# chanzuckerberg/saber

Measured on AMD Instinct MI355X. Metric: EM slices/sec (1024^2, Hiera-L), higher is better.
Workload: dtype bf16; 1 GPU; 1024x1024 uint16 EM slice -> prep.prepare -> SAM2 AMG (Hiera-L, cfgAMG defaults: npoints=32, crop_n_layers=2 -> 21 crops, 3072 grid prompts + 9216 m2m refinements, multimask) -> dedup/sort -> uint16 label plane; BASELINE configs[1]; weights=seeded synthetic Hiera-L (no checkpoint offline), slices_per_rank=22, engine_handles_per_gpu=2, parallelism=single GPU

## Files before the change

### include/saber_amd_kernels.h

```cpp
#ifndef SABER_AMD_KERNELS_H
#define SABER_AMD_KERNELS_H
#include <stdint.h>
#ifdef __cplusplus
extern "C" {
#endif

const char* saber_k_last_error(void);
int saber_k_init(int device_id);

int saber_k_gemm(const uint16_t* A, const uint16_t* W, const float* bias, const float* res, float* out_f32, uint16_t* out_bf16,
                 int M, int N, int K, int act, int act_last, int pool4, int res_shift, int res_mod, void* stream);

int saber_k_gemm_ld(const uint16_t* A, int lda, const uint16_t* W, int ldw, int w_kpad, const float* bias, const float* res, float* out_f32,
                    uint16_t* out_bf16, int M, int N, int K, int act, void* stream);

int saber_k_gemm_rowln(const uint16_t* A, int lda, const uint16_t* W, int ldw, const float* bias, const float* res, float* out_f32,
                       uint16_t* out_bf16, const float* ln_gamma, const float* ln_beta, float ln_eps, uint16_t* ln_out, int M, int N, int K,
                       void* stream);

int saber_k_mlp_rowln(const uint16_t* A, int lda, const uint16_t* W1, int ldw1, const float* b1, const uint16_t* W2, int ldw2, const float* b2,
                      const float* res, float* out_f32, uint16_t* out_bf16, const float* ln_gamma, const float* ln_beta, float ln_eps,
                      uint16_t* ln_out, int M, int C, void* stream);

int saber_k_layernorm(const float* x, const float* gamma, const float* beta, float eps, float* out_f32, uint16_t* out_bf16,
                      int rows, int C, int act, void* stream);

int saber_k_hiera_attention(const uint16_t* qkv, uint16_t* out, int n_windows, int nk, int heads, int q_pool, void* stream);
int saber_k_hiera_attention_ex(const uint16_t* qkv, uint16_t* out, int n_windows, int nk, int heads, int head_dim, int q_pool,
                               const uint8_t* key_mask, void* stream);

int saber_k_dec_attention(const float* q, const float* k, const float* v, uint16_t* out, int B, int nq, int nk, int heads, int hd,
                          int k_shared, void* stream);

int saber_k_prepare(const void* img, int dtype, int H, int W, float* out, float* ws_dev, uint32_t* minmax_dev, void* stream);

int saber_k_mask_post(const float* lowres, int n, int crop_x0, int crop_y0, int crop_w, int crop_h, int H, int W, float thr,
                      float offset, uint32_t* bits, int32_t* stats, void* stream);
// ... 92 lines not shown
```

### saber_amd/_lib.py

```python
import ctypes as C
import os
import subprocess

_HERE = os.path.dirname(os.path.abspath(__file__))
LIB_PATH = os.path.join(_HERE, "libsaber_amd.so")
CSRC = os.path.join(_HERE, "csrc")


class SaberAmdError(RuntimeError):
    pass


class SaberRangeError(SaberAmdError):
    """SABER_ERR_RANGE: the engine's overflow sentinel found NaN / inf in the 16-bit arithmetic (include/saber_amd.h:
    saber_engine_check_finite) - with fp16 operands, an activation beyond 65 504.  The call's results are invalid."""


SABER_OK, SABER_ERR_INVALID, SABER_ERR_STATE, SABER_ERR_HIP, SABER_ERR_CAPACITY, SABER_ERR_RANGE = 0, -1, -2, -3, -4, -5


def build(verbose: bool = False) -> str:
    r = subprocess.run(["make", "-C", CSRC, "-j8"], capture_output=True, text=True)
    if r.returncode != 0:
        raise SaberAmdError("building libsaber_amd.so failed:\n" + r.stdout[-4000:] + r.stderr[-4000:])
# ... 76 lines not shown
    "saber_classifier_predict": (_i, [_vp, _vp, _i, _i, _vp, _i, _i, _vp, _vp]),
    "saber_classifier_predict_bits": (_i, [_vp, _vp, _i, _i, _vp, _i, C.POINTER(_i), _i, _i, _vp, _vp]),
    "saber_classifier_head": (_i, [_vp, _vp, _i, _vp, _vp]),
    "saber_classifier_get_crops": (_i, [_vp, _i, _vp, _vp, _vp]),
    "saber_profile_begin": (_i, [_vp]),
    "saber_profile_end": (_i, [_vp, C.POINTER(ProfileClass), _i]),
    "saber_encoder_flops": (C.c_double, [_vp]),
    "saber_decoder_flops_per_prompt": (C.c_double, []),
    "saber_k_last_error": (C.c_char_p, []),
    "saber_k_init": (_i, [_i]),
    "saber_k_gemm": (_i, [_vp, _vp, _vp, _vp, _vp, _vp, _i, _i, _i, _i, _i, _i, _i, _i, _vp]),
    "saber_k_gemm_ld": (_i, [_vp, _i, _vp, _i, _i, _vp, _vp, _vp, _vp, _i, _i, _i, _i, _vp]),
    "saber_k_gemm_rowln": (_i, [_vp, _i, _vp, _i, _vp, _vp, _vp, _vp, _vp, _vp, _f, _vp, _i, _i, _i, _vp]),
    "saber_k_mlp_rowln": (_i, [_vp, _i, _vp, _i, _vp, _vp, _i, _vp, _vp, _vp, _vp, _vp, _vp, _f, _vp, _i, _i, _vp]),
    "saber_k_layernorm": (_i, [_vp, _vp, _vp, _f, _vp, _vp, _i, _i, _i, _vp]),
    "saber_k_hiera_attention": (_i, [_vp, _vp, _i, _i, _i, _i, _vp]),
    "saber_k_hiera_attention_ex": (_i, [_vp, _vp, _i, _i, _i, _i, _i, _vp, _vp]),
    "saber_k_dec_attention": (_i, [_vp, _vp, _vp, _vp, _i, _i, _i, _i, _i, _i, _vp]),
    "saber_k_prepare": (_i, [_vp, _i, _i, _i, _vp, _vp, _vp, _vp]),
    "saber_k_mask_post": (_i, [_vp, _i, _i, _i, _i, _i, _i, _i, _f, _f, _vp, _vp, _vp]),
    "saber_k_perm_index": (_i, [_i, _i, _i]),
    "saber_k_set_operand_type": (_i, [_i]),
    "saber_k_stream_create_cu_range": (_i, [_i, _i, C.POINTER(_vp)]),
    "saber_k_stream_destroy": (_i, [_vp]),
    "saber_k_host_f32_to_f16": (None, [_vp, _vp, C.c_int64]),
    "saber_k_dec_i2t": (_i, [_vp, C.c_int64, _vp, _vp, _vp, _f, _vp, _vp, _vp, _vp, _vp, _f, _vp, _i, _vp]),
    "saber_k_dec_i2t16": (_i, [_vp, C.c_int64, _vp, _vp, _vp, _f, _vp, _vp, _vp, _vp, _vp, _f, _vp, _i, _i, _vp]),
    "saber_k_dec_t2i": (_i, [_vp, C.c_int64, _vp, _vp, _vp, _f, _vp, _vp, _i, _i, _vp, _vp, _vp, _vp]),
    "saber_k_dec_upscale": (_i, [_vp, _vp, _vp, _vp, _vp, _vp, _vp, _vp, _vp, _i, _i, _vp, _vp, _i, _vp, _vp, _i, _vp, _vp]),
    "saber_k_mask_pick": (_i, [_vp, _vp, _i, _i, _vp, _vp, _vp, _vp]),
# ... 68 lines not shown
```

### saber_amd/csrc/capi_kernels.hip

```cpp
#include <cmath>
#include <cstring>
#include <string>
#include <vector>

#include "../../include/saber_amd_kernels.h"
#include "common.h"
#include "kernels.h"
#include "engine.h"
#include "exact.h"

#include <atomic>

static thread_local std::string g_kerr;
static int kfail(const char* m) { g_kerr = m ? m : "unknown"; return -1; }
static int kcheck(const char* m) {
    if (m) return kfail(m);
    hipError_t st = hipGetLastError();
    if (st != hipSuccess) return kfail(hipGetErrorString(st));
    return 0;
}

extern "C" const char* saber_k_last_error(void) { return g_kerr.c_str(); }

extern "C" int saber_k_init(int device_id) {
    if (hipSetDevice(device_id) != hipSuccess) return kfail("hipSetDevice failed");
    const char* m = gemm_init_device();
    if (!m) m = gemm_rowln_init_device();
    if (!m) m = gemm_mlp_rowln_init_device();
    if (!m) m = hiera_attention_init_device();
    if (!m) m = image_ops_init_device();
    if (!m) m = decoder_fused_init_device();
    if (!m) m = decoder_t16_init_device();
    if (!m) m = amg_device_init();
    (void)hipGetLastError();
    if (m) return kfail(m);
    return 0;
}

extern "C" int saber_k_gemm(const uint16_t* A, const uint16_t* W, const float* bias, const float* res, float* out_f32,
                            uint16_t* out_bf16, int M, int N, int K, int act, int act_last, int pool4, int res_shift, int res_mod,
                            void* stream) {
    GemmParams p;
    p.A = A; p.lda = K; p.W = W; p.ldw = K; p.bias = bias; p.res = res; p.ldres = N; p.Cf = out_f32; p.ldcf = N; p.Cb = out_bf16; p.ldcb = N;
// ... 44 lines not shown
                                 int M, int C, void* stream) {
    if (!gemm_mlp_rowln_width(C)) return kfail("mlp_rowln: width not built (C must be 144)");
    static thread_local bf16_t* scratch = nullptr;
    static thread_local size_t scratch_elems = 0;
    const size_t need = gemm_mlp_rowln_packed_elems(C);
    if (need > scratch_elems) {
        if (scratch) { (void)hipDeviceSynchronize(); (void)hipFree(scratch); scratch = nullptr; scratch_elems = 0; }
        if (hipMalloc(reinterpret_cast<void**>(&scratch), need * sizeof(bf16_t)) != hipSuccess) return kfail("mlp_rowln: scratch allocation failed");
        scratch_elems = need;
    }
    if (const char* m = launch_pack_mlp_chunks(W1, ldw1, W2, ldw2, C, scratch, (hipStream_t)stream)) return kfail(m);
    GemmParams p;
    p.A = A; p.lda = lda; p.bias1 = b1; p.bias = b2; p.res = res; p.ldres = C; p.Cf = out_f32; p.ldcf = C; p.Cb = out_bf16; p.ldcb = C;
    p.M = M; p.N = C; p.K = C; p.ln_gamma = ln_gamma; p.ln_beta = ln_beta; p.ln_eps = ln_eps; p.ln_out = ln_out; p.ldln = C; p.Wpk = scratch;
    return kcheck(launch_gemm_mlp_rowln(p, (hipStream_t)stream));
}

extern "C" int saber_k_layernorm(const float* x, const float* gamma, const float* beta, float eps, float* out_f32, uint16_t* out_bf16,
                                 int rows, int C, int act, void* stream) {
    LayerNormParams p;
    p.x = x; p.ldx = C; p.gamma = gamma; p.beta = beta; p.eps = eps; p.out_f = out_f32; p.out_bf = out_bf16; p.ldo = C; p.rows = rows; p.C = C; p.act = act;
    return kcheck(launch_layernorm(p, (hipStream_t)stream));
}

extern "C" int saber_k_hiera_attention(const uint16_t* qkv, uint16_t* out, int n_windows, int nk, int heads, int q_pool, void* stream) {
    return kcheck(launch_hiera_attention(qkv, out, n_windows, nk, heads, 72, q_pool, nullptr, (hipStream_t)stream));
}

extern "C" int saber_k_hiera_attention_ex(const uint16_t* qkv, uint16_t* out, int n_windows, int nk, int heads, int head_dim, int q_pool,
                                          const uint8_t* key_mask, void* stream) {
// ... 301 lines not shown
```

### saber_amd/csrc/engine.hip

```cpp
#include "engine.h"

#include <algorithm>
#include <cmath>
#include <cstring>
#include <functional>
#include <utility>

#include "common.h"

static thread_local std::string g_create_err;

int eng_fail(saber_engine* e, int code, const std::string& msg) {
    if (e) e->err = msg; else g_create_err = msg;
    return code;
}

int eng_alloc_bytes(saber_engine* e, void** p, size_t bytes) {
    *p = nullptr;
    if (bytes == 0) bytes = 16;
    hipError_t st = hipMalloc(p, bytes);
    if (st != hipSuccess) return eng_fail(e, SABER_ERR_HIP, std::string("hipMalloc(") + std::to_string(bytes) + "): " + hipGetErrorString(st));
    e->allocs.push_back(*p);
    return SABER_OK;
}
// ... 162 lines not shown
    int ndev = 0;
    if (hipGetDeviceCount(&ndev) != hipSuccess || ndev <= 0) return eng_fail(nullptr, SABER_ERR_HIP, "no HIP device visible: the MI355X engine cannot run");
    if (device_id < 0 || device_id >= ndev) return eng_fail(nullptr, SABER_ERR_INVALID, "device_id out of range");
    if (hipSetDevice(device_id) != hipSuccess) return eng_fail(nullptr, SABER_ERR_HIP, "hipSetDevice failed");
    saber_engine* e = new saber_engine();
    e->device = device_id;
    e->trunk = t;
    e->max_images = max_images;
    e->max_prompts = max_prompts;
    if (const char* g = getenv("SABER_AMD_GRAPHS")) e->graphs_on = atoi(g) != 0;
    if (const char* m = hiera_spec(e, *spec)) { delete e; return eng_fail(nullptr, SABER_ERR_INVALID, m); }
    {
        const char* m = gemm_init_device();
            if (!m) m = gemm_rowln_init_device();
            if (!m) m = gemm_mlp_rowln_init_device();
        if (!m) m = amg_device_init();
        if (!m) m = hiera_attention_init_device();
        if (!m) m = image_ops_init_device();
        if (!m) m = decoder_fused_init_device();
        if (!m) m = decoder_tokens_init_device();
        if (!m) m = decoder_t16_init_device();
        (void)hipGetLastError();
        if (m) { delete e; return eng_fail(nullptr, SABER_ERR_HIP, std::string("kernel attribute setup: ") + m); }
    }
    *out = e;
    return SABER_OK;
}

extern "C" void saber_engine_destroy(saber_engine* e) {
    if (!e) return;
// ... 693 lines not shown
    }
    if (!e->crops_pin) ENG_HIP(e, hipHostMalloc(reinterpret_cast<void**>(&e->crops_pin), sizeof(int) * 256 * 8));
    const int* src = crops_host;
    int slot = 0;
    if (crops_host != e->crops_pin) {
        slot = e->crops_next;
        e->crops_next = slot == 7 ? 1 : slot + 1;
        if (!e->crops_ev[slot]) ENG_HIP(e, hipEventCreateWithFlags(&e->crops_ev[slot], hipEventDisableTiming));
        else ENG_HIP(e, hipEventSynchronize(e->crops_ev[slot]));
        memcpy(e->crops_pin + 256 * slot, crops_host, sizeof(int) * 4 * n);
        src = e->crops_pin + 256 * slot;
    }
    ENG_HIP(e, hipMemcpyAsync(e->crops_dev, src, sizeof(int) * 4 * n, hipMemcpyHostToDevice, s));
    if (slot) ENG_HIP(e, hipEventRecord(e->crops_ev[slot], s));
    ENG_KP(e, PC_IMAGE, 0.0, 0.0, launch_resize_normalize(img_dev, H, W, channels, e->crops_dev, n, e->pix, 1024, s));
    ENG_KP(e, PC_IMAGE, 0.0, 0.0, launch_patch_embed(e->pix, e->pe_wt, e->pe_bias, e->pos_table, e->xa, n, e->embed_dim, 1024, s));
    if (e->precision == SABER_PRECISION_EXACT) {
        TRY(exact_encode_blocks(e, n, slot0, s));
        for (int i = 0; i < n; ++i) { e->slot_valid[slot0 + i] = 1; e->slot_shared_valid[slot0 + i] = 0; e->slot_embb_valid[slot0 + i] = 0; }
        return SABER_OK;
    }
    float* x = e->xa;
    float* xalt = e->xb;
    int tokens = 65536;
    int stage = 0;
    static const bool no_rowln = getenv("SABER_AMD_NO_ROWLN") != nullptr;
    const bool fuse = !e->padded && !no_rowln;
    static const bool no_mlpfuse = getenv("SABER_AMD_NO_MLPFUSE") != nullptr;
    const bool mlpfuse = fuse && !no_mlpfuse && !(g_saber_debug_flags & 262144);
    const size_t nblocks = e->blocks.size();
    ENG_KP(e, PC_LAYERNORM, 0.0, 0.0, ln_run(x, e->bw[0].n1, 1e-6f, n * tokens, e->blocks[0].din, nullptr, e->xn, ACT_NONE, s, nullptr, nullptr, 0, e->valid[0], tokens));
    const int snake = (g_saber_debug_flags & 512) ? 0 : 1;
    uint8_t* const xn8 = reinterpret_cast<uint8_t*>(e->xn);
    uint8_t* const hid8 = reinterpret_cast<uint8_t*>(e->hid);
    for (size_t i = 0; i < nblocks; ++i) {
        const BlockSpec& bs = e->blocks[i];
        const BlockW& w = e->bw[i];
        const int N = n * tokens;
        float* xres = x;
        int Nq = N;
        if (bs.din != bs.dout) {
            GemmParams g = mk_gemm(e->xn, bs.din, N, w.sc);
            g.Cf = xalt; g.ldcf = bs.dout; g.pool4 = 1;
            ENG_KP(e, PC_GEMM, 2.0 * g.M * (double)g.N * g.K * g.batch, gemm_bytes(g), launch_gemm(g, s));
            xres = xalt;
            Nq = N / 4;
// ... 635 lines not shown
```

### saber_amd/csrc/gemm_mlp_rowln.hip

```cpp
#include "common.h"
#include "kernels.h"
#include "rowln_epilogue.h"

#define ML_HC 32

template <int C> struct MlpRowLnCfg {
    static_assert(C == 144, "built for the stage-0 width");
    static constexpr int R = 256;
    static constexpr int NK1 = (C + 31) / 32;
    static constexpr int NT = C / 16;
    static constexpr int FR = 2 * NK1 + NT;
    static constexpr int NCH = 4 * C / ML_HC;
    static constexpr int CHUNK = FR * 1024;
    static constexpr int UNITS = CHUNK / 16, NU = (UNITS + 511) / 512;
    static constexpr int BUF = NU * 512 * 16;
    static constexpr int B1_OFF = 2 * BUF;
    static constexpr int SCR_OFF = B1_OFF + 4 * C * 4;
    static constexpr int LDS = SCR_OFF + 8 * RL_SCR;
};

template <int C>
__global__ __launch_bounds__(512) void gemm_rowln_mlp_kernel(GemmParams p) {
    using CF = MlpRowLnCfg<C>;
    constexpr int R = CF::R, NK1 = CF::NK1, NT = CF::NT, NCH = CF::NCH, NU = CF::NU;
    static_assert(NT == 9, "rowln_epilogue: 9 column tiles per wave");
    extern __shared__ __attribute__((aligned(16))) char smem[];
    const int tid = threadIdx.x, lane = tid & 63;
    const int wave = __builtin_amdgcn_readfirstlane(tid >> 6);
    const int fi = lane & 15, fg = lane >> 4;
    const int tiles = (p.M + R - 1) / R;
    int tl = blockIdx.x;
    if (tl >= tiles) return;
    auto tile_of = [&](int l) { return p.rev ? tiles - 1 - l : l; };

    float* b1s = reinterpret_cast<float*>(smem + CF::B1_OFF);
    for (int i = tid; i < 4 * C; i += 512) b1s[i] = p.bias1 ? p.bias1[i] : 0.f;

    const u32x4* __restrict__ wsrc = reinterpret_cast<const u32x4*>(p.Wpk);
    u32x4 st[NU];
    auto stage_load = [&](int ch) {
#pragma unroll
        for (int q = 0; q < NU; ++q) st[q] = wsrc[(int64_t)ch * CF::UNITS + min(tid + 512 * q, CF::UNITS - 1)];
    };
    auto stage_write = [&](int buf) {
#pragma unroll
        for (int q = 0; q < NU; ++q) *reinterpret_cast<u32x4*>(smem + buf * CF::BUF + (tid + 512 * q) * 16) = st[q];
    };
    op16x8 xn[2][NK1];
    auto load_xn = [&](int tile) {
        const int rows = min(R, p.M - tile * R);
        const __amdgpu_buffer_rsrc_t arsrc = __builtin_amdgcn_make_buffer_rsrc((void*)(p.A + (int64_t)tile * R * p.lda), 0, (int)((uint32_t)rows * (uint32_t)p.lda * 2u), 0x00020000);
        const uint32_t voff = (uint32_t)(((wave * 32 + fi) * (int)p.lda + fg * 8) * 2);
        const uint32_t istep = (uint32_t)(16 * (int)p.lda * 2);
#pragma unroll
        for (int i = 0; i < 2; ++i)
#pragma unroll
            for (int ks = 0; ks < NK1; ++ks) {
                u32x4 v = __builtin_amdgcn_raw_buffer_load_b128(arsrc, voff + ks * 64, i * istep, 0);
                if ((ks + 1) * 32 > C && ks * 32 + fg * 8 >= C) v = (u32x4){0u, 0u, 0u, 0u};
                xn[i][ks] = __builtin_bit_cast(op16x8, v);
            }
// ... 72 lines not shown
    }
}

bool gemm_mlp_rowln_width(int C) { return C == 144; }
size_t gemm_mlp_rowln_packed_elems(int C) { return (size_t)(4 * C / ML_HC) * (2 * ((C + 31) / 32) + C / 16) * 512; }
const char* launch_pack_mlp_chunks(const bf16_t* W1, int ldw1, const bf16_t* W2, int ldw2, int C, bf16_t* out, hipStream_t s) {
    if (!gemm_mlp_rowln_width(C)) return "pack_mlp_chunks: width not built (144)";
    if ((ldw1 & 7) || ldw1 < C || (ldw2 & 7) || ldw2 < 4 * C) return "pack_mlp_chunks: ldw1 / ldw2 must be multiples of 8 and cover the rows";
    if (((uintptr_t)W1 & 15) || ((uintptr_t)W2 & 15) || ((uintptr_t)out & 15)) return "pack_mlp_chunks: operand alignment";
    const int total = (int)(gemm_mlp_rowln_packed_elems(C) / 8);
    hipLaunchKernelGGL(pack_mlp_chunks_kernel, dim3((unsigned)((total + 255) / 256)), dim3(256), 0, s, W1, ldw1, W2, ldw2, C, out);
    return nullptr;
}

const char* gemm_mlp_rowln_init_device() {
    const hipError_t st = hipFuncSetAttribute(reinterpret_cast<const void*>(gemm_rowln_mlp_kernel<144>), hipFuncAttributeMaxDynamicSharedMemorySize, MlpRowLnCfg<144>::LDS);
    return st == hipSuccess ? nullptr : hipGetErrorString(st);
}

const char* launch_gemm_mlp_rowln(const GemmParams& p_in, hipStream_t stream) {
    GemmParams p = p_in;
    p.dbg = g_saber_debug_flags;
    if (!gemm_mlp_rowln_width(p.N) || p.K != p.N || !p.Wpk || !p.Cf || !p.ln_out || !p.ln_gamma || !p.ln_beta || p.batch > 1 || p.pool4 || p.act != ACT_NONE ||
        p.res_shift || p.res_mod)
        return "gemm_mlp_rowln: unsupported problem (C must be 144; packed weights, fp32 + LayerNorm outputs required)";
    if (p.M <= 0) return "gemm_mlp_rowln: empty problem";
    if (p.lda & 7) return "gemm_mlp_rowln: lda must be a multiple of 8";
    if (((uintptr_t)p.A & 15) || ((uintptr_t)p.Wpk & 15) || ((uintptr_t)p.Cf & 15) || (p.ldcf & 3) || ((uintptr_t)p.ln_out & 7) || (p.ldln & 3) ||
        (p.res && (((uintptr_t)p.res & 15) || (p.ldres & 3))) || (p.bias && ((uintptr_t)p.bias & 15)) || (p.bias1 && ((uintptr_t)p.bias1 & 3)) ||
        (p.Cb && (((uintptr_t)p.Cb & 7) || (p.ldcb & 3))) || ((uintptr_t)p.ln_gamma & 15) || ((uintptr_t)p.ln_beta & 15))
        return "gemm_mlp_rowln: operand alignment";
    if ((int64_t)p.M * p.lda >= ((int64_t)1 << 40)) return "gemm_mlp_rowln: problem too large";
    const int n_cu = saber_cu_count();
    const int tiles = (p.M + MlpRowLnCfg<144>::R - 1) / MlpRowLnCfg<144>::R;
    hipLaunchKernelGGL((gemm_rowln_mlp_kernel<144>), dim3(tiles < n_cu ? tiles : n_cu), dim3(512), MlpRowLnCfg<144>::LDS, stream, p);
    return nullptr;
}
```

### saber_amd/csrc/kernels.h

```cpp
#pragma once
#include <hip/hip_runtime.h>
#include <stdint.h>
#include <stddef.h>

extern int g_saber_debug_flags;
extern unsigned long long* g_saber_stamp_buf;
int saber_cu_count();
extern thread_local int g_saber_op_f16;
inline bool saber_op_is_f16() { return g_saber_op_f16 != 0; }

typedef uint16_t bf16_t;

enum { ACT_NONE = 0, ACT_GELU = 1, ACT_RELU = 2, ACT_SIGMOID = 3 };

struct GemmParams {
    const bf16_t* A = nullptr; int64_t lda = 0; int64_t strideA = 0;
    const bf16_t* W = nullptr; int64_t ldw = 0; int64_t strideW = 0;
    const float* bias = nullptr; int64_t strideBias = 0;
    const float* res = nullptr; int64_t ldres = 0; int64_t strideRes = 0;
    float* Cf = nullptr; int64_t ldcf = 0; int64_t strideCf = 0;
    bf16_t* Cb = nullptr; int64_t ldcb = 0; int64_t strideCb = 0;
    int M = 0, N = 0, K = 0;
    int act = ACT_NONE;
    int act_last = 0;
// ... 115 lines not shown

namespace op_bf16 {
#include "kernels_op.h"
}
namespace op_f16 {
#include "kernels_op.h"
}
#ifndef SABER_OP_NS
#define SABER_OP_FWD(fn)                                                                                                  \
    template <class... A> inline auto fn(A&&... a) {                                                                      \
        return saber_op_is_f16() ? op_f16::fn(static_cast<A&&>(a)...) : op_bf16::fn(static_cast<A&&>(a)...);              \
    }
#define SABER_OP_INIT(fn)                                                                                                 \
    inline const char* fn() { const char* m = op_bf16::fn(); return m ? m : op_f16::fn(); }
SABER_OP_INIT(gemm_init_device) SABER_OP_INIT(gemm_rowln_init_device) SABER_OP_INIT(gemm_mlp_rowln_init_device) SABER_OP_INIT(hiera_attention_init_device)
SABER_OP_INIT(decoder_fused_init_device) SABER_OP_INIT(decoder_tokens_init_device) SABER_OP_INIT(decoder_t16_init_device)
SABER_OP_FWD(launch_gemm) SABER_OP_FWD(gemm_rowln_supported) SABER_OP_FWD(launch_gemm_rowln) SABER_OP_FWD(gemm_rowln_packed_elems) SABER_OP_FWD(launch_pack_w_kstep)
SABER_OP_FWD(gemm_mlp_rowln_width) SABER_OP_FWD(gemm_mlp_rowln_packed_elems) SABER_OP_FWD(launch_pack_mlp_chunks) SABER_OP_FWD(launch_gemm_mlp_rowln)
SABER_OP_FWD(launch_layernorm) SABER_OP_FWD(launch_gather_rows) SABER_OP_FWD(launch_add_to_bf16) SABER_OP_FWD(launch_hiera_attention)
SABER_OP_FWD(launch_prompt_tokens) SABER_OP_FWD(launch_prompt_tokens_multi) SABER_OP_FWD(launch_mask_embed_src) SABER_OP_FWD(launch_mask_hidden) SABER_OP_FWD(launch_embb_tiles)
SABER_OP_FWD(launch_dec_attention) SABER_OP_FWD(launch_mask_pick) SABER_OP_FWD(launch_iou_live_flags) SABER_OP_FWD(launch_mask_select)
SABER_OP_FWD(launch_dec_fold) SABER_OP_FWD(launch_dec_t2i) SABER_OP_FWD(launch_dec_i2t) SABER_OP_FWD(launch_dec_i2t_t2i) SABER_OP_FWD(launch_dec_upscale) SABER_OP_FWD(launch_dec_tokens)
SABER_OP_FWD(launch_prompt_tokens16) SABER_OP_FWD(launch_dec_tokens16) SABER_OP_FWD(launch_dec_i2t16)
SABER_OP_FWD(launch_mask_post) SABER_OP_FWD(launch_gather_masks) SABER_OP_FWD(launch_label_plane) SABER_OP_FWD(launch_pair_intersections) SABER_OP_FWD(launch_unpermute_nchw)
SABER_OP_FWD(launch_rope) SABER_OP_FWD(launch_softmax_rows) SABER_OP_FWD(launch_conv3x3s2) SABER_OP_FWD(launch_unpack_masks) SABER_OP_FWD(launch_paint_nearest)
SABER_OP_FWD(launch_conv3x3s2_t) SABER_OP_FWD(launch_dwconv7_t) SABER_OP_FWD(launch_dwconv7) SABER_OP_FWD(launch_conv4x4s4) SABER_OP_FWD(launch_resize_plane)
SABER_OP_FWD(launch_flash256) SABER_OP_FWD(launch_gauss_mirror) SABER_OP_FWD(launch_axpy) SABER_OP_FWD(launch_bf16_to_f32)
SABER_OP_FWD(launch_rope_batched) SABER_OP_FWD(launch_flash256_batched) SABER_OP_FWD(launch_membank_assemble)
#undef SABER_OP_FWD
#undef SABER_OP_INIT
#endif
```

### saber_amd/csrc/kernels_op.h

```cpp
const char* launch_gemm(const GemmParams& p, hipStream_t stream);
const char* gemm_init_device();
bool gemm_rowln_supported(const GemmParams& p);
const char* launch_gemm_rowln(const GemmParams& p, hipStream_t stream);
const char* gemm_rowln_init_device();
size_t gemm_rowln_packed_elems(int N, int K);
const char* launch_pack_w_kstep(const bf16_t* W, int ldw, int N, int K, bf16_t* out, hipStream_t s);
bool gemm_mlp_rowln_width(int C);
size_t gemm_mlp_rowln_packed_elems(int C);
const char* launch_pack_mlp_chunks(const bf16_t* W1, int ldw1, const bf16_t* W2, int ldw2, int C, bf16_t* out, hipStream_t s);
const char* launch_gemm_mlp_rowln(const GemmParams& p, hipStream_t stream);
const char* gemm_mlp_rowln_init_device();
const char* launch_layernorm(const LayerNormParams& p, hipStream_t s);
const char* launch_gather_rows(const float* in, int64_t in_rows, float* out, int64_t out_rows, const int* idx, int C, int n_images, hipStream_t s);
const char* launch_add_to_bf16(const float* x, const float* y, int ymod, bf16_t* out_bf, float* out_f, int64_t rows, int C,
                               hipStream_t s);
const char* launch_hiera_attention(const bf16_t* qkv, bf16_t* out, int n_windows, int nk, int heads, int hd, int q_pool,
                                   const uint8_t* kmask, hipStream_t s);
const char* hiera_attention_init_device();
const char* launch_prompt_tokens(const float* pts, const int* labels, int P, PromptWeights w, float* tokens, hipStream_t s);
const char* launch_prompt_tokens_multi(const float* pts, const int* labels, int P, int K, PromptWeights w, float* tokens, hipStream_t s);
const char* launch_mask_embed_src(const float* mask_in, int P, const float* image_embed, XMap emb_map, const float* pos, MaskEmbedWeights w,
                                  float* src_f, bf16_t* src_bf, bf16_t* srcpos_bf, float clamp_abs, hipStream_t s, int raw4_q0 = -1);
const char* launch_mask_hidden(const float* mask_in, int P, MaskEmbedWeights w, bf16_t* h2, float clamp_abs, hipStream_t s, int raw4_q0 = -1);
const char* launch_embb_tiles(const float* emb, const float* b3, float* out, hipStream_t s);
const char* launch_dec_attention(const float* q, const float* k, const float* v, bf16_t* out, int B, int nq, int nk, int heads,
                                 int hd, int64_t q_bs, int64_t k_bs, int64_t v_bs, int64_t o_bs, hipStream_t s);
const char* launch_mask_pick(const float* masks4, const float* iou4, int P, int multimask, float* out_iou, int* out_sel, hipStream_t s, const uint8_t* live = nullptr);
// ... 50 lines not shown
```

### saber_amd/csrc/layernorm.hip

```cpp
#include <algorithm>

#include "common.h"
#include "kernels.h"

#define LN_MAX_CHUNKS 5

template <int NCH>
__global__ __launch_bounds__(256) void layernorm_kernel(LayerNormParams p) {
    const int lane = threadIdx.x & 63;
    const int64_t n_waves = (int64_t)gridDim.x * 4;
    const int64_t row0 = (int64_t)blockIdx.x * 4 + (threadIdx.x >> 6);
    if (row0 >= p.rows) return;
    const int nvec = p.C >> 2;
    float4 g[NCH], b[NCH];
#pragma unroll
    for (int i = 0; i < NCH; ++i) {
        const int c = lane + 64 * i;
        if (c < nvec) { g[i] = *reinterpret_cast<const float4*>(p.gamma + 4 * c); b[i] = *reinterpret_cast<const float4*>(p.beta + 4 * c); }
        else { g[i] = make_float4(0.f, 0.f, 0.f, 0.f); b[i] = g[i]; }
    }
    const float invC = 1.0f / (float)p.C;
    float4 v[NCH], vn[NCH];
    auto load_row = [&](int64_t row, float4 (&dst)[NCH]) {
        const float* x = p.x + row * p.ldx;
// ... 64 lines not shown
    float4 v[3], vn[3];
    auto load_row = [&](int64_t grp, float4 (&dst)[3]) {
        const int64_t row = grp * 4 + sub;
        const float* x = p.x + (row < p.rows ? row : (int64_t)p.rows - 1) * p.ldx;
#pragma unroll
        for (int i = 0; i < 3; ++i) {
            const int c = li + 16 * i;
            dst[i] = c < nvec ? *reinterpret_cast<const float4*>(x + 4 * c) : make_float4(0.f, 0.f, 0.f, 0.f);
        }
    };
    if (g0 >= n_row_groups) return;
    load_row(g0, v);
    for (int64_t grp = g0; grp < n_row_groups; grp += n_groups) {
        if (grp + n_groups < n_row_groups) load_row(grp + n_groups, vn);
        const int64_t row = grp * 4 + sub;
        float s = 0.f;
#pragma unroll
        for (int i = 0; i < 3; ++i) s += (v[i].x + v[i].y) + (v[i].z + v[i].w);
        const float mean = row16_sum(s) * invC;
        float q = 0.f;
#pragma unroll
        for (int i = 0; i < 3; ++i) {
            if (li + 16 * i < nvec) {
                const float a = v[i].x - mean, bb = v[i].y - mean, cc = v[i].z - mean, d = v[i].w - mean;
                q += (a * a + bb * bb) + (cc * cc + d * d);
            }
        }
        const float rstd = 1.0f / sqrtf(row16_sum(q) * invC + p.eps);
        if (row < p.rows) {
            const float* addv = p.addvec ? p.addvec + (int64_t)(row % p.add_mod) * p.C : nullptr;
            const bool zero_row = p.row_valid && !p.row_valid[row % p.valid_mod];
#pragma unroll
            for (int i = 0; i < 3; ++i) {
                const int c = li + 16 * i;
                if (c < nvec) {
                    float y0 = (v[i].x - mean) * rstd * g[i].x + b[i].x;
                    float y1 = (v[i].y - mean) * rstd * g[i].y + b[i].y;
                    float y2 = (v[i].z - mean) * rstd * g[i].z + b[i].z;
                    float y3 = (v[i].w - mean) * rstd * g[i].w + b[i].w;
                    if (p.act == ACT_GELU) { y0 = gelu_erf(y0); y1 = gelu_erf(y1); y2 = gelu_erf(y2); y3 = gelu_erf(y3); }
                    if (zero_row) { y0 = 0.f; y1 = 0.f; y2 = 0.f; y3 = 0.f; }
                    if (p.out_f) *reinterpret_cast<float4*>(p.out_f + row * p.ldo + 4 * c) = make_float4(y0, y1, y2, y3);
                    if (p.out_bf)
                        *reinterpret_cast<uint2*>(p.out_bf + row * p.ldo + 4 * c) = make_uint2(pack_op16(y0, y1), pack_op16(y2, y3));
                    if (p.out_bf_add) {
                        const float4 a = *reinterpret_cast<const float4*>(addv + 4 * c);
                        *reinterpret_cast<uint2*>(p.out_bf_add + row * p.ldo + 4 * c) =
                            make_uint2(pack_op16(y0 + a.x, y1 + a.y), pack_op16(y2 + a.z, y3 + a.w));
                    }
                }
            }
        }
#pragma unroll
        for (int i = 0; i < 3; ++i) v[i] = vn[i];
// ... 91 lines not shown
```

Baseline: 7.532 slices/s.

## Fuse Hiera patch embedding with first-block LayerNorm in an MFMA kernel

Adds a patch_embed_ln kernel that computes the 7x7 stride-4 patch embedding with fp32 MFMA, adds bias and positional embedding, and applies the first block's LayerNorm in the same pass. It writes both the fp32 residual stream and the 16-bit normalized activations, so the separate LayerNorm launch over all stage-0 tokens is skipped. The MLP row-LN kernel is also templated on wave count, with an opt-in 4-wave, two-workgroups-per-CU variant behind an environment flag. The fused path is specialized to embed dim 144 at 1024 resolution, and can be turned off by an environment variable or a debug flag.

Result: no change. 7.518 slices/s, median of 2 (-0.2%).

```diff
diff --git a/include/saber_amd_kernels.h b/include/saber_amd_kernels.h
--- a/include/saber_amd_kernels.h
+++ b/include/saber_amd_kernels.h
@@ -21,6 +21,10 @@
 int saber_k_mlp_rowln(const uint16_t* A, int lda, const uint16_t* W1, int ldw1, const float* b1, const uint16_t* W2, int ldw2, const float* b2,
                       const float* res, float* out_f32, uint16_t* out_bf16, const float* ln_gamma, const float* ln_beta, float ln_eps,
                       uint16_t* ln_out, int M, int C, void* stream);
+
+int saber_k_patch_embed(const float* pix, const float* wt, const float* bias, const float* pos, float* out, int n_images, int C, void* stream);
+int saber_k_patch_embed_ln(const float* pix, const float* wt, const float* bias, const float* pos, const float* ln_gamma, const float* ln_beta,
+                           float ln_eps, float* out, uint16_t* ln_out, int n_images, int C, void* stream);
 
 int saber_k_layernorm(const float* x, const float* gamma, const float* beta, float eps, float* out_f32, uint16_t* out_bf16,
                       int rows, int C, int act, void* stream);
diff --git a/saber_amd/_lib.py b/saber_amd/_lib.py
--- a/saber_amd/_lib.py
+++ b/saber_amd/_lib.py
@@ -114,6 +114,8 @@
     "saber_k_gemm_rowln": (_i, [_vp, _i, _vp, _i, _vp, _vp, _vp, _vp, _vp, _vp, _f, _vp, _i, _i, _i, _vp]),
     "saber_k_mlp_rowln": (_i, [_vp, _i, _vp, _i, _vp, _vp, _i, _vp, _vp, _vp, _vp, _vp, _vp, _f, _vp, _i, _i, _vp]),
     "saber_k_layernorm": (_i, [_vp, _vp, _vp, _f, _vp, _vp, _i, _i, _i, _vp]),
+    "saber_k_patch_embed": (_i, [_vp, _vp, _vp, _vp, _vp, _i, _i, _vp]),
+    "saber_k_patch_embed_ln": (_i, [_vp, _vp, _vp, _vp, _vp, _vp, _f, _vp, _vp, _i, _i, _vp]),
     "saber_k_hiera_attention": (_i, [_vp, _vp, _i, _i, _i, _i, _vp]),
     "saber_k_hiera_attention_ex": (_i, [_vp, _vp, _i, _i, _i, _i, _i, _vp, _vp]),
     "saber_k_dec_attention": (_i, [_vp, _vp, _vp, _vp, _i, _i, _i, _i, _i, _i, _vp]),
diff --git a/saber_amd/csrc/capi_kernels.hip b/saber_amd/csrc/capi_kernels.hip
--- a/saber_amd/csrc/capi_kernels.hip
+++ b/saber_amd/csrc/capi_kernels.hip
@@ -27,6 +27,7 @@
     const char* m = gemm_init_device();
     if (!m) m = gemm_rowln_init_device();
     if (!m) m = gemm_mlp_rowln_init_device();
+    if (!m) m = patch_embed_ln_init_device();
     if (!m) m = hiera_attention_init_device();
     if (!m) m = image_ops_init_device();
     if (!m) m = decoder_fused_init_device();
@@ -101,6 +102,15 @@
     p.A = A; p.lda = lda; p.bias1 = b1; p.bias = b2; p.res = res; p.ldres = C; p.Cf = out_f32; p.ldcf = C; p.Cb = out_bf16; p.ldcb = C;
     p.M = M; p.N = C; p.K = C; p.ln_gamma = ln_gamma; p.ln_beta = ln_beta; p.ln_eps = ln_eps; p.ln_out = ln_out; p.ldln = C; p.Wpk = scratch;
     return kcheck(launch_gemm_mlp_rowln(p, (hipStream_t)stream));
+}
+
+extern "C" int saber_k_patch_embed(const float* pix, const float* wt, const float* bias, const float* pos, float* out, int n_images, int C, void* stream) {
+    return kcheck(launch_patch_embed(pix, wt, bias, pos, out, n_images, C, 1024, (hipStream_t)stream));
+}
+
+extern "C" int saber_k_patch_embed_ln(const float* pix, const float* wt, const float* bias, const float* pos, const float* ln_gamma, const float* ln_beta,
+                                      float ln_eps, float* out, uint16_t* ln_out, int n_images, int C, void* stream) {
+    return kcheck(launch_patch_embed_ln(pix, wt, bias, pos, ln_gamma, ln_beta, ln_eps, out, ln_out, n_images, C, 1024, (hipStream_t)stream));
 }
 
 extern "C" int saber_k_layernorm(const float* x, const float* gamma, const float* beta, float eps, float* out_f32, uint16_t* out_bf16,
diff --git a/saber_amd/csrc/engine.hip b/saber_amd/csrc/engine.hip
--- a/saber_amd/csrc/engine.hip
+++ b/saber_amd/csrc/engine.hip
@@ -200,6 +200,7 @@
         const char* m = gemm_init_device();
             if (!m) m = gemm_rowln_init_device();
             if (!m) m = gemm_mlp_rowln_init_device();
+            if (!m) m = patch_embed_ln_init_device();
         if (!m) m = amg_device_init();
         if (!m) m = hiera_attention_init_device();
         if (!m) m = image_ops_init_device();
@@ -923,7 +924,14 @@
     ENG_HIP(e, hipMemcpyAsync(e->crops_dev, src, sizeof(int) * 4 * n, hipMemcpyHostToDevice, s));
     if (slot) ENG_HIP(e, hipEventRecord(e->crops_ev[slot], s));
     ENG_KP(e, PC_IMAGE, 0.0, 0.0, launch_resize_normalize(img_dev, H, W, channels, e->crops_dev, n, e->pix, 1024, s));
-    ENG_KP(e, PC_IMAGE, 0.0, 0.0, launch_patch_embed(e->pix, e->pe_wt, e->pe_bias, e->pos_table, e->xa, n, e->embed_dim, 1024, s));
+    static const bool no_entryfuse = getenv("SABER_AMD_NO_ENTRYFUSE") != nullptr;
+    const bool entryfuse = e->precision != SABER_PRECISION_EXACT && !e->padded && patch_embed_ln_supported(e->embed_dim, 1024) &&
+                           e->blocks[0].din == e->embed_dim && !no_entryfuse && !(g_saber_debug_flags & 524288);
+    if (entryfuse)
+        ENG_KP(e, PC_IMAGE, 0.0, 0.0, launch_patch_embed_ln(e->pix, e->pe_wt, e->pe_bias, e->pos_table, e->bw[0].n1.g, e->bw[0].n1.b, 1e-6f, e->xa, e->xn, n,
+                                                            e->embed_dim, 1024, s));
+    else
+        ENG_KP(e, PC_IMAGE, 0.0, 0.0, launch_patch_embed(e->pix, e->pe_wt, e->pe_bias, e->pos_table, e->xa, n, e->embed_dim, 1024, s));
     if (e->precision == SABER_PRECISION_EXACT) {
         TRY(exact_encode_blocks(e, n, slot0, s));
         for (int i = 0; i < n; ++i) { e->slot_valid[slot0 + i] = 1; e->slot_shared_valid[slot0 + i] = 0; e->slot_embb_valid[slot0 + i] = 0; }
@@ -938,7 +946,8 @@
     static const bool no_mlpfuse = getenv("SABER_AMD_NO_MLPFUSE") != nullptr;
     const bool mlpfuse = fuse && !no_mlpfuse && !(g_saber_debug_flags & 262144);
     const size_t nblocks = e->blocks.size();
-    ENG_KP(e, PC_LAYERNORM, 0.0, 0.0, ln_run(x, e->bw[0].n1, 1e-6f, n * tokens, e->blocks[0].din, nullptr, e->xn, ACT_NONE, s, nullptr, nullptr, 0, e->valid[0], tokens));
+    if (!entryfuse)
+        ENG_KP(e, PC_LAYERNORM, 0.0, 0.0, ln_run(x, e->bw[0].n1, 1e-6f, n * tokens, e->blocks[0].din, nullptr, e->xn, ACT_NONE, s, nullptr, nullptr, 0, e->valid[0], tokens));
     const int snake = (g_saber_debug_flags & 512) ? 0 : 1;
     uint8_t* const xn8 = reinterpret_cast<uint8_t*>(e->xn);
     uint8_t* const hid8 = reinterpret_cast<uint8_t*>(e->hid);
diff --git a/saber_amd/csrc/gemm_mlp_rowln.hip b/saber_amd/csrc/gemm_mlp_rowln.hip
--- a/saber_amd/csrc/gemm_mlp_rowln.hip
+++ b/saber_amd/csrc/gemm_mlp_rowln.hip
@@ -4,24 +4,26 @@
 
 #define ML_HC 32
 
-template <int C> struct MlpRowLnCfg {
+template <int C, int NW> struct MlpRowLnCfg {
     static_assert(C == 144, "built for the stage-0 width");
-    static constexpr int R = 256;
+    static constexpr int NTHR = 64 * NW;
+    static constexpr int R = 32 * NW;
     static constexpr int NK1 = (C + 31) / 32;
     static constexpr int NT = C / 16;
     static constexpr int FR = 2 * NK1 + NT;
     static constexpr int NCH = 4 * C / ML_HC;
     static constexpr int CHUNK = FR * 1024;
-    static constexpr int UNITS = CHUNK / 16, NU = (UNITS + 511) / 512;
-    static constexpr int BUF = NU * 512 * 16;
+    static constexpr int UNITS = CHUNK / 16, NU = (UNITS + NTHR - 1) / NTHR;
+    static constexpr int BUF = NU * NTHR * 16;
     static constexpr int B1_OFF = 2 * BUF;
     static constexpr int SCR_OFF = B1_OFF + 4 * C * 4;
-    static constexpr int LDS = SCR_OFF + 8 * RL_SCR;
+    static constexpr int LDS = SCR_OFF + NW * RL_SCR;
 };
 
-template <int C>
-__global__ __launch_bounds__(512) void gemm_rowln_mlp_kernel(GemmParams p) {
-    using CF = MlpRowLnCfg<C>;
+template <int C, int NW>
+__global__ __launch_bounds__(64 * NW, 2) void gemm_rowln_mlp_kernel(GemmParams p) {
+    using CF = MlpRowLnCfg<C, NW>;
+    constexpr int NTHR = CF::NTHR;
     constexpr int R = CF::R, NK1 = CF::NK1, NT = CF::NT, NCH = CF::NCH, NU = CF::NU;
     static_assert(NT == 9, "rowln_epilogue: 9 column tiles per wave");
     extern __shared__ __attribute__((aligned(16))) char smem[];
@@ -34,17 +36,17 @@
     auto tile_of = [&](int l) { return p.rev ? tiles - 1 - l : l; };
 
     float* b1s = reinterpret_cast<float*>(smem + CF::B1_OFF);
-    for (int i = tid; i < 4 * C; i += 512) b1s[i] = p.bias1 ? p.bias1[i] : 0.f;
+    for (int i = tid; i < 4 * C; i += NTHR) b1s[i] = p.bias1 ? p.bias1[i] : 0.f;
 
     const u32x4* __restrict__ wsrc = reinterpret_cast<const u32x4*>(p.Wpk);
     u32x4 st[NU];
     auto stage_load = [&](int ch) {
 #pragma unroll
-        for (int q = 0; q < NU; ++q) st[q] = wsrc[(int64_t)ch * CF::UNITS + min(tid + 512 * q, CF::UNITS - 1)];
+        for (int q = 0; q < NU; ++q) st[q] = wsrc[(int64_t)ch * CF::UNITS + min(tid + NTHR * q, CF::UNITS - 1)];
     };
     auto stage_write = [&](int buf) {
 #pragma unroll
-        for (int q = 0; q < NU; ++q) *reinterpret_cast<u32x4*>(smem + buf * CF::BUF + (tid + 512 * q) * 16) = st[q];
+        for (int q = 0; q < NU; ++q) *reinterpret_cast<u32x4*>(smem + buf * CF::BUF + (tid + NTHR * q) * 16) = st[q];
     };
     op16x8 xn[2][NK1];
     auto load_xn = [&](int tile) {
@@ -147,7 +149,9 @@
 }
 
 const char* gemm_mlp_rowln_init_device() {
-    const hipError_t st = hipFuncSetAttribute(reinterpret_cast<const void*>(gemm_rowln_mlp_kernel<144>), hipFuncAttributeMaxDynamicSharedMemorySize, MlpRowLnCfg<144>::LDS);
+    hipError_t st = hipFuncSetAttribute(reinterpret_cast<const void*>(gemm_rowln_mlp_kernel<144, 8>), hipFuncAttributeMaxDynamicSharedMemorySize, MlpRowLnCfg<144, 8>::LDS);
+    if (st == hipSuccess)
+        st = hipFuncSetAttribute(reinterpret_cast<const void*>(gemm_rowln_mlp_kernel<144, 4>), hipFuncAttributeMaxDynamicSharedMemorySize, MlpRowLnCfg<144, 4>::LDS);
     return st == hipSuccess ? nullptr : hipGetErrorString(st);
 }
 
@@ -165,7 +169,16 @@
         return "gemm_mlp_rowln: operand alignment";
     if ((int64_t)p.M * p.lda >= ((int64_t)1 << 40)) return "gemm_mlp_rowln: problem too large";
     const int n_cu = saber_cu_count();
-    const int tiles = (p.M + MlpRowLnCfg<144>::R - 1) / MlpRowLnCfg<144>::R;
-    hipLaunchKernelGGL((gemm_rowln_mlp_kernel<144>), dim3(tiles < n_cu ? tiles : n_cu), dim3(512), MlpRowLnCfg<144>::LDS, stream, p);
+    static const bool waves4 = getenv("SABER_AMD_MLP_WAVES4") != nullptr;
+    if (waves4 || (p.dbg & 256)) {
+        using CF = MlpRowLnCfg<144, 4>;
+        static_assert(2 * CF::LDS <= 160 * 1024, "two workgroups per CU");
+        const int tiles = (p.M + CF::R - 1) / CF::R;
+        hipLaunchKernelGGL((gemm_rowln_mlp_kernel<144, 4>), dim3(tiles < 2 * n_cu ? tiles : 2 * n_cu), dim3(CF::NTHR), CF::LDS, stream, p);
+    } else {
+        using CF = MlpRowLnCfg<144, 8>;
+        const int tiles = (p.M + CF::R - 1) / CF::R;
+        hipLaunchKernelGGL((gemm_rowln_mlp_kernel<144, 8>), dim3(tiles < n_cu ? tiles : n_cu), dim3(CF::NTHR), CF::LDS, stream, p);
+    }
     return nullptr;
 }
diff --git a/saber_amd/csrc/kernels.h b/saber_amd/csrc/kernels.h
--- a/saber_amd/csrc/kernels.h
+++ b/saber_amd/csrc/kernels.h
@@ -153,7 +153,7 @@
 #define SABER_OP_INIT(fn)                                                                                                 \
     inline const char* fn() { const char* m = op_bf16::fn(); return m ? m : op_f16::fn(); }
 SABER_OP_INIT(gemm_init_device) SABER_OP_INIT(gemm_rowln_init_device) SABER_OP_INIT(gemm_mlp_rowln_init_device) SABER_OP_INIT(hiera_attention_init_device)
-SABER_OP_INIT(decoder_fused_init_device) SABER_OP_INIT(decoder_tokens_init_device) SABER_OP_INIT(decoder_t16_init_device)
+SABER_OP_INIT(decoder_fused_init_device) SABER_OP_INIT(decoder_tokens_init_device) SABER_OP_INIT(decoder_t16_init_device) SABER_OP_INIT(patch_embed_ln_init_device)
 SABER_OP_FWD(launch_gemm) SABER_OP_FWD(gemm_rowln_supported) SABER_OP_FWD(launch_gemm_rowln) SABER_OP_FWD(gemm_rowln_packed_elems) SABER_OP_FWD(launch_pack_w_kstep)
 SABER_OP_FWD(gemm_mlp_rowln_width) SABER_OP_FWD(gemm_mlp_rowln_packed_elems) SABER_OP_FWD(launch_pack_mlp_chunks) SABER_OP_FWD(launch_gemm_mlp_rowln)
 SABER_OP_FWD(launch_layernorm) SABER_OP_FWD(launch_gather_rows) SABER_OP_FWD(launch_add_to_bf16) SABER_OP_FWD(launch_hiera_attention)
@@ -165,6 +165,7 @@
 SABER_OP_FWD(launch_rope) SABER_OP_FWD(launch_softmax_rows) SABER_OP_FWD(launch_conv3x3s2) SABER_OP_FWD(launch_unpack_masks) SABER_OP_FWD(launch_paint_nearest)
 SABER_OP_FWD(launch_conv3x3s2_t) SABER_OP_FWD(launch_dwconv7_t) SABER_OP_FWD(launch_dwconv7) SABER_OP_FWD(launch_conv4x4s4) SABER_OP_FWD(launch_resize_plane)
 SABER_OP_FWD(launch_flash256) SABER_OP_FWD(launch_gauss_mirror) SABER_OP_FWD(launch_axpy) SABER_OP_FWD(launch_bf16_to_f32)
+SABER_OP_FWD(patch_embed_ln_supported) SABER_OP_FWD(launch_patch_embed_ln)
 SABER_OP_FWD(launch_rope_batched) SABER_OP_FWD(launch_flash256_batched) SABER_OP_FWD(launch_membank_assemble)
 #undef SABER_OP_FWD
 #undef SABER_OP_INIT
diff --git a/saber_amd/csrc/kernels_op.h b/saber_amd/csrc/kernels_op.h
--- a/saber_amd/csrc/kernels_op.h
+++ b/saber_amd/csrc/kernels_op.h
@@ -11,6 +11,10 @@
 const char* launch_gemm_mlp_rowln(const GemmParams& p, hipStream_t stream);
 const char* gemm_mlp_rowln_init_device();
 const char* launch_layernorm(const LayerNormParams& p, hipStream_t s);
+bool patch_embed_ln_supported(int C, int res);
+const char* launch_patch_embed_ln(const float* pix, const float* wt, const float* bias, const float* pos, const float* gamma, const float* beta, float eps,
+                                  float* out, bf16_t* out_ln, int n_images, int C, int res, hipStream_t s);
+const char* patch_embed_ln_init_device();
 const char* launch_gather_rows(const float* in, int64_t in_rows, float* out, int64_t out_rows, const int* idx, int C, int n_images, hipStream_t s);
 const char* launch_add_to_bf16(const float* x, const float* y, int ymod, bf16_t* out_bf, float* out_f, int64_t rows, int C,
                                hipStream_t s);
diff --git a/saber_amd/csrc/layernorm.hip b/saber_amd/csrc/layernorm.hip
--- a/saber_amd/csrc/layernorm.hip
+++ b/saber_amd/csrc/layernorm.hip
@@ -2,6 +2,7 @@
 
 #include "common.h"
 #include "kernels.h"
+#include "layernorm_rows4.h"
 
 #define LN_MAX_CHUNKS 5
 
@@ -102,19 +103,8 @@
     for (int64_t grp = g0; grp < n_row_groups; grp += n_groups) {
         if (grp + n_groups < n_row_groups) load_row(grp + n_groups, vn);
         const int64_t row = grp * 4 + sub;
-        float s = 0.f;
-#pragma unroll
-        for (int i = 0; i < 3; ++i) s += (v[i].x + v[i].y) + (v[i].z + v[i].w);
-        const float mean = row16_sum(s) * invC;
-        float q = 0.f;
-#pragma unroll
-        for (int i = 0; i < 3; ++i) {
-            if (li + 16 * i < nvec) {
-                const float a = v[i].x - mean, bb = v[i].y - mean, cc = v[i].z - mean, d = v[i].w - mean;
-                q += (a * a + bb * bb) + (cc * cc + d * d);
-            }
-        }
-        const float rstd = 1.0f / sqrtf(row16_sum(q) * invC + p.eps);
+        float mean, rstd;
+        ln_row16_stats(v, li, nvec, invC, p.eps, &mean, &rstd);
         if (row < p.rows) {
             const float* addv = p.addvec ? p.addvec + (int64_t)(row % p.add_mod) * p.C : nullptr;
             const bool zero_row = p.row_valid && !p.row_valid[row % p.valid_mod];
@@ -122,10 +112,8 @@
             for (int i = 0; i < 3; ++i) {
                 const int c = li + 16 * i;
                 if (c < nvec) {
-                    float y0 = (v[i].x - mean) * rstd * g[i].x + b[i].x;
-                    float y1 = (v[i].y - mean) * rstd * g[i].y + b[i].y;
-                    float y2 = (v[i].z - mean) * rstd * g[i].z + b[i].z;
-                    float y3 = (v[i].w - mean) * rstd * g[i].w + b[i].w;
+                    const float4 y = ln_row16_apply(v[i], mean, rstd, g[i], b[i]);
+                    float y0 = y.x, y1 = y.y, y2 = y.z, y3 = y.w;
                     if (p.act == ACT_GELU) { y0 = gelu_erf(y0); y1 = gelu_erf(y1); y2 = gelu_erf(y2); y3 = gelu_erf(y3); }
                     if (zero_row) { y0 = 0.f; y1 = 0.f; y2 = 0.f; y3 = 0.f; }
                     if (p.out_f) *reinterpret_cast<float4*>(p.out_f + row * p.ldo + 4 * c) = make_float4(y0, y1, y2, y3);
diff --git a/saber_amd/csrc/layernorm_rows4.h b/saber_amd/csrc/layernorm_rows4.h
--- /dev/null
+++ b/saber_amd/csrc/layernorm_rows4.h
@@ -0,0 +1,23 @@
+#pragma once
+#include "common.h"
+
+__device__ __forceinline__ void ln_row16_stats(const float4 (&v)[3], int li, int nvec, float invC, float eps, float* mean_out, float* rstd_out) {
+    float s = 0.f;
+#pragma unroll
+    for (int i = 0; i < 3; ++i) s += (v[i].x + v[i].y) + (v[i].z + v[i].w);
+    const float mean = row16_sum(s) * invC;
+    float q = 0.f;
+#pragma unroll
+    for (int i = 0; i < 3; ++i) {
+        if (li + 16 * i < nvec) {
+            const float a = v[i].x - mean, bb = v[i].y - mean, cc = v[i].z - mean, d = v[i].w - mean;
+            q += (a * a + bb * bb) + (cc * cc + d * d);
+        }
+    }
+    *mean_out = mean;
+    *rstd_out = 1.0f / sqrtf(row16_sum(q) * invC + eps);
+}
+
+__device__ __forceinline__ float4 ln_row16_apply(const float4& v, float mean, float rstd, const float4& g, const float4& b) {
+    return make_float4((v.x - mean) * rstd * g.x + b.x, (v.y - mean) * rstd * g.y + b.y, (v.z - mean) * rstd * g.z + b.z, (v.w - mean) * rstd * g.w + b.w);
+}
diff --git a/saber_amd/csrc/patch_embed_ln.hip b/saber_amd/csrc/patch_embed_ln.hip
--- /dev/null
+++ b/saber_amd/csrc/patch_embed_ln.hip
@@ -0,0 +1,167 @@
+#include "common.h"
+#include "kernels.h"
+#include "layernorm_rows4.h"
+
+#define PEL_C 144
+#define PEL_KS 37
+#define PEL_W_FLOATS (PEL_KS * 9 * 64)
+#define PEL_PATCH_FLOATS (3 * 35 * 36)
+#define PEL_PATCH_LOADS 15
+#define PEL_ST_PITCH 148
+#define PEL_LDS ((PEL_W_FLOATS + 2 * PEL_PATCH_FLOATS + 4 * 16 * PEL_ST_PITCH) * 4)
+
+__device__ __forceinline__ void pel_barrier() { asm volatile("s_waitcnt lgkmcnt(0)\n\ts_barrier" ::: "memory"); }
+
+__global__ __launch_bounds__(256) void patch_embed_ln_kernel(const float* __restrict__ pix, const float* __restrict__ wt, const float* __restrict__ bias,
+                                                             const float* __restrict__ pos, const float* __restrict__ gamma, const float* __restrict__ beta,
+                                                             float eps, float* __restrict__ out, bf16_t* __restrict__ out_ln, int n_images, int res) {
+    extern __shared__ __attribute__((aligned(16))) char smem[];
+    float* const Wl = reinterpret_cast<float*>(smem);
+    float* const patch = Wl + PEL_W_FLOATS;
+    const int tid = threadIdx.x, lane = tid & 63;
+    const int wave = __builtin_amdgcn_readfirstlane(tid >> 6);
+    const int fi = lane & 15, fg = lane >> 4;
+    float* const stage = patch + 2 * PEL_PATCH_FLOATS + wave * (16 * PEL_ST_PITCH);
+    const int64_t plane = (int64_t)res * res;
+
+    for (int idx = tid; idx < 148 * 36; idx += 256) {
+        const int k = idx / 36, cq = idx - k * 36;
+        const float4 v = k < 147 ? *reinterpret_cast<const float4*>(wt + k * PEL_C + cq * 4) : make_float4(0.f, 0.f, 0.f, 0.f);
+        *reinterpret_cast<float4*>(Wl + ((k >> 2) * 9 + (cq >> 2)) * 64 + (k & 3) * 16 + (cq & 3) * 4) = v;
+    }
+    const int t = wave * 16 + fi;
+    const int ty = (((t >> 5) & 1) << 2) | (((t >> 3) & 1) << 1) | ((t >> 1) & 1);
+    const int tx = (((t >> 4) & 1) << 2) | (((t >> 2) & 1) << 1) | (t & 1);
+    int poff[PEL_KS];
+#pragma unroll
+    for (int ks = 0; ks < PEL_KS; ++ks) {
+        const int k = ks * 4 + fg < 147 ? ks * 4 + fg : 0;
+        const int c = k / 49, r = k - c * 49, ky = r / 7, kx = r - ky * 7;
+        poff[ks] = c * (35 * 36) + (ty * 4 + ky) * 36 + tx * 4 + kx;
+    }
+    int loff[PEL_PATCH_LOADS];
+#pragma unroll
+    for (int q = 0; q < PEL_PATCH_LOADS; ++q) {
+        const int idx = tid + 256 * q;
+        const int c = idx / 1225, r = idx - c * 1225, py = r / 35, px = r - py * 35;
+        loff[q] = idx < 3 * 35 * 35 ? c * (35 * 36) + py * 36 + px : 35;
+    }
+    float4 b4[9];
+#pragma unroll
+    for (int ct = 0; ct < 9; ++ct) b4[ct] = *reinterpret_cast<const float4*>(bias + ct * 16 + fg * 4);
+    const int sub = fg, li = fi;
+    float4 g[3], bt[3];
+#pragma unroll
+    for (int i = 0; i < 3; ++i) {
+        const int c = li + 16 * i;
+        if (c < PEL_C / 4) { g[i] = *reinterpret_cast<const float4*>(gamma + 4 * c); bt[i] = *reinterpret_cast<const float4*>(beta + 4 * c); }
+        else { g[i] = make_float4(0.f, 0.f, 0.f, 0.f); bt[i] = g[i]; }
+    }
+    const float invC = 1.0f / (float)PEL_C;
+
+    int cur = 0;
+    for (int wi = blockIdx.x; wi < 1024; wi += gridDim.x) {
+        int wy, wx;
+        perm_coords256(wi * 64, &wy, &wx);
+        const int iy0 = wy * 4 - 3, ix0 = wx * 4 - 3;
+        int goff[PEL_PATCH_LOADS];
+#pragma unroll
+        for (int q = 0; q < PEL_PATCH_LOADS; ++q) {
+            const int idx = tid + 256 * q;
+            const int c = idx / 1225, r = idx - c * 1225, py = r / 35, px = r - py * 35;
+            const int iy = iy0 + py, ix = ix0 + px;
+            goff[q] = (idx < 3 * 35 * 35 && iy >= 0 && iy < res && ix >= 0 && ix < res) ? c * (int)plane + iy * res + ix : -1;
+        }
+        float pr[PEL_PATCH_LOADS];
+        auto load_patch = [&](int b) {
+            const float* pb = pix + (int64_t)b * 3 * plane;
+#pragma unroll
+            for (int q = 0; q < PEL_PATCH_LOADS; ++q) pr[q] = pb[max(goff[q], 0)];
+        };
+        auto write_patch = [&](int buf) {
+#pragma unroll
+            for (int q = 0; q < PEL_PATCH_LOADS; ++q) patch[buf * PEL_PATCH_FLOATS + loff[q]] = goff[q] >= 0 ? pr[q] : 0.f;
+        };
+        load_patch(0);
+        const int64_t row0 = (int64_t)wi * 64 + wave * 16;
+        float4 p4[9];
+#pragma unroll
+        for (int ct = 0; ct < 9; ++ct) p4[ct] = *reinterpret_cast<const float4*>(pos + (row0 + fi) * PEL_C + ct * 16 + fg * 4);
+        write_patch(cur);
+        pel_barrier();
+        for (int b = 0; b < n_images; ++b) {
+            load_patch(b + 1 < n_images ? b + 1 : b);
+            __builtin_amdgcn_sched_barrier(0);
+            const float* pb = patch + cur * PEL_PATCH_FLOATS;
+            f32x4 acc[9];
+#pragma unroll
+            for (int ct = 0; ct < 9; ++ct) acc[ct] = (f32x4){0.f, 0.f, 0.f, 0.f};
+            float wa[2][9], pv[2];
+            auto load_step = [&](int ks, float (&w)[9], float& v) {
+                v = pb[poff[ks]];
+#pragma unroll
+                for (int ct = 0; ct < 9; ++ct) w[ct] = Wl[(ks * 9 + ct) * 64 + lane];
+            };
+            load_step(0, wa[0], pv[0]);
+#pragma unroll
+            for (int ks = 0; ks < PEL_KS; ++ks) {
+                if (ks + 1 < PEL_KS) load_step(ks + 1, wa[(ks + 1) & 1], pv[(ks + 1) & 1]);
+                __builtin_amdgcn_sched_barrier(0);
+#pragma unroll
+                for (int ct = 0; ct < 9; ++ct) acc[ct] = __builtin_amdgcn_mfma_f32_16x16x4f32(wa[ks & 1][ct], pv[ks & 1], acc[ct], 0, 0, 0);
+                __builtin_amdgcn_sched_barrier(0);
+            }
+            write_patch(cur ^ 1);
+#pragma unroll
+            for (int ct = 0; ct < 9; ++ct)
+                *reinterpret_cast<float4*>(stage + fi * PEL_ST_PITCH + ct * 16 + fg * 4) =
+                    make_float4(acc[ct][0] + b4[ct].x + p4[ct].x, acc[ct][1] + b4[ct].y + p4[ct].y, acc[ct][2] + b4[ct].z + p4[ct].z, acc[ct][3] + b4[ct].w + p4[ct].w);
+            const int64_t orow0 = (int64_t)b * 65536 + row0;
+#pragma unroll
+            for (int ps = 0; ps < 4; ++ps) {
+                const int rl = ps * 4 + sub;
+                float4 v[3];
+#pragma unroll
+                for (int i = 0; i < 3; ++i) {
+                    const int c = li + 16 * i;
+                    v[i] = c < PEL_C / 4 ? *reinterpret_cast<const float4*>(stage + rl * PEL_ST_PITCH + 4 * c) : make_float4(0.f, 0.f, 0.f, 0.f);
+                }
+                float mean, rstd;
+                ln_row16_stats(v, li, PEL_C / 4, invC, eps, &mean, &rstd);
+                float* of = out + (orow0 + rl) * PEL_C;
+                bf16_t* ol = out_ln + (orow0 + rl) * PEL_C;
+#pragma unroll
+                for (int i = 0; i < 3; ++i) {
+                    const int c = li + 16 * i;
+                    if (c < PEL_C / 4) {
+                        const float4 y = ln_row16_apply(v[i], mean, rstd, g[i], bt[i]);
+                        *reinterpret_cast<float4*>(of + 4 * c) = v[i];
+                        *reinterpret_cast<uint2*>(ol + 4 * c) = make_uint2(pack_op16(y.x, y.y), pack_op16(y.z, y.w));
+                    }
+                }
+            }
+            pel_barrier();
+            cur ^= 1;
+        }
+    }
+}
+
+const char* patch_embed_ln_init_device() {
+    const hipError_t st = hipFuncSetAttribute(reinterpret_cast<const void*>(patch_embed_ln_kernel), hipFuncAttributeMaxDynamicSharedMemorySize, PEL_LDS);
+    return st == hipSuccess ? nullptr : hipGetErrorString(st);
+}
+
+bool patch_embed_ln_supported(int C, int res) { return C == PEL_C && res == 1024; }
+
+const char* launch_patch_embed_ln(const float* pix, const float* wt, const float* bias, const float* pos, const float* gamma, const float* beta, float eps,
+                                  float* out, bf16_t* out_ln, int n_images, int C, int res, hipStream_t s) {
+    if (!patch_embed_ln_supported(C, res)) return "patch_embed_ln: built for embed dim 144 at 1024x1024 model input";
+    if (n_images <= 0) return nullptr;
+    if (!pix || !wt || !bias || !pos || !gamma || !beta || !out || !out_ln) return "patch_embed_ln: null pointer";
+    if (((uintptr_t)wt & 15) || ((uintptr_t)bias & 15) || ((uintptr_t)pos & 15) || ((uintptr_t)gamma & 15) || ((uintptr_t)beta & 15) || ((uintptr_t)out & 15) ||
+        ((uintptr_t)out_ln & 7) || ((uintptr_t)pix & 3))
+        return "patch_embed_ln: operand alignment";
+    const int n_cu = saber_cu_count();
+    hipLaunchKernelGGL(patch_embed_ln_kernel, dim3(n_cu < 1024 ? n_cu : 1024), dim3(256), PEL_LDS, s, pix, wt, bias, pos, gamma, beta, eps, out, out_ln, n_images, res);
+    return nullptr;
+}
```
